# MoayedHajiAli/ElasticDiffusion-official

Hardware: AMD Instinct MI355X
Metric: images/sec at 50 steps (SDXL 2048x1024) (higher is better)
Workload: dtype fp16

## Files before the change

elasticdiffusion_official_amd/_hip.py:

```python
import ctypes
import os
import subprocess

import torch

PKG_DIR = os.path.dirname(os.path.abspath(__file__))
ROOT_DIR = os.path.dirname(PKG_DIR)
SOURCES = [os.path.join(PKG_DIR, "csrc", n) for n in ("elastic_kernels.hip", "unet_kernels.hip", "attention_kernels.hip", "gemm_kernels.hip", "vae_kernels.hip",
                                                       "canny_kernels.hip", "resize_kernels.hip", "mask_kernels.hip", "lora_kernels.hip")]
SRC = SOURCES[0]
INCLUDE = os.path.join(ROOT_DIR, "include")
SO_PATH = os.path.join(PKG_DIR, "libelastic_hip.so")
ABI_VERSION = 13

HIPCC_FLAGS = ["--offload-arch=gfx950", "-O3", "-std=c++17", "-ffp-contract=off", "-fPIC", "-shared"]

_i32p = ctypes.POINTER(ctypes.c_int32)
_vp, _i, _f, _i64 = ctypes.c_void_p, ctypes.c_int, ctypes.c_float, ctypes.c_int64

SIGNATURES = {
    "ed_version": [],
    "ed_error_string": [_i],
    "ed_gather_views": [_vp, _vp, _i, _i, _i, _i, _i, _vp, _vp, _i, _i, _i, _i, _i, _i, _i, _vp, _f, _vp],
    "ed_scatter_centres": [_vp, _i, _vp, _i, _i, _i, _i, _i, _i, _i, _vp, _vp, _vp, _vp, _vp],
# ... 21 lines not shown
    "ed_groupnorm_nhwc_cat": [_vp, _vp, _vp, _vp, _vp, _vp, _i, _i, _i, _i, _i, _i, _f, _i, _vp],
    "ed_assemble_rows": [_vp, _i, _i, _i, _i, _vp, _vp, _vp, _vp, _vp, _vp, _i, _i, _i, _i, _i, _i, _i, _vp, _vp, _vp, _vp,
                         _i, _i, _i, _i, _i, _i, _i, _i, _vp],
    "ed_assemble_rows_x": [_vp, _i, _i, _i, _i, _vp, _vp, _vp, _vp, _vp, _vp, _i, _i, _i, _i, _i, _i, _i, _vp, _vp, _vp, _vp,
                           _i, _i, _i, _i, _i, _i, _i, _i, _vp, _i, _vp, _vp],
    "ed_phase_epilogue": [_vp, _vp, _i, _vp, _vp, _vp, _vp, _vp, _vp, _vp, _vp, _vp, _vp, _vp, _vp, _vp, _vp, _vp, _vp, _vp,
                          _vp, _vp, _vp, _i, _i, _i, _i, _i, _i, _i, _i, _i, _i, _i, _i, _i, _i, _f, _f, _f, _f, _f, _f, _f,
                          _vp],
    "ed_softmax_rows": [_vp, _i64, _i64, _f, _vp],
    "ed_groupnorm_f32": [_vp, _vp, _vp, _vp, _vp, _i, _i, _i, _i, _f, _i, _vp],
    "ed_groupnorm_f32_workspace": [_i, _i, _i, _i],
    "ed_flash_attention": [_vp, _vp, _vp, _vp, _i, _i, _i, _i, _i, _i, _i64, _i64, _i64, _i64, _i64, _i64, _i64, _i64, _f, _i, _vp],
    "ed_geglu_gemm": [_vp, _vp, _vp, _vp, _i, _i64, _i, _i, _vp],
    "ed_linear": [_vp, _vp, _vp, _vp, _vp, _i, _i64, _i, _i, _vp],
    "ed_conv3x3_nhwc": [_vp, _vp, _vp, _vp, _vp, _vp, _i, _i, _i, _i, _i, _i, _vp],
    "ed_conv3x3_nhwc_up2x": [_vp, _vp, _vp, _vp, _i, _i, _i, _i, _i, _i, _vp],
    "ed_conv3x3_nhwc_s2": [_vp, _vp, _vp, _vp, _i, _i, _i, _i, _i, _i, _vp],
    "ed_absmax_f32": [_vp, _i64, _vp, _vp],
    "ed_split_f32_nhwc": [_vp, _vp, _i, _i, _i, _i, _i, _vp, _vp],
    "ed_groupnorm_nhwc_f32_workspace": [_i, _i, _i, _i],
    "ed_groupnorm_nhwc_f32": [_vp, _vp, _vp, _vp, _vp, _i, _i, _i, _i, _f, _i, _i, _vp],
    "ed_conv3x3_nhwc_f32out": [_vp, _vp, _vp, _vp, _vp, _i, _i, _i, _i, _i, _i, _f, _vp, _vp],
    "ed_conv3x3_nhwc_f32out_s2": [_vp, _vp, _vp, _vp, _i, _i, _i, _i, _i, _i, _f, _vp, _vp],
    "ed_canny_workspace": [_i, _i, _i],
    "ed_canny_map": [_vp, _i, _i, _i, _i, _i, _vp, _vp],
    "ed_canny_hysteresis": [_vp, _i, _i, _vp, _vp, _vp],
    "ed_canny_edges": [_vp, _i, _i, _vp, _vp, _vp],
    "ed_cfg_ddim_step_pt": [_vp, _vp, _vp, _vp, _vp, _f, _f, _f, _f, _f, _i64, _i, _vp],
    "ed_rrg_update_pt": [_vp, _vp, _vp, _vp, _vp, _vp, _vp, _vp, _f, _f, _f, _f, _f, _i, _i, _i, _i, _i, _i, _i, _vp],
    "ed_phase_epilogue_pt": [_vp, _vp, _i, _vp, _vp, _vp, _vp, _vp, _vp, _vp, _vp, _vp, _vp, _vp, _vp, _vp, _vp, _vp, _vp,
# ... 81 lines not shown
```

elasticdiffusion_official_amd/csrc/gemm_kernels.hip:

```cpp
#include <hip/hip_runtime.h>
#include <stdint.h>
#include <stdlib.h>

#include "elastic_hip.h"

namespace {

typedef float f32x4 __attribute__((ext_vector_type(4)));
typedef __bf16 bf16x8 __attribute__((ext_vector_type(8)));
typedef _Float16 f16x8 __attribute__((ext_vector_type(8)));
typedef uint32_t u32x4 __attribute__((ext_vector_type(4)));
typedef __attribute__((address_space(3))) void* lds_ptr_t;

struct BF {
  typedef bf16x8 v8;
  static __device__ __forceinline__ f32x4 mfma(v8 a, v8 b, f32x4 c) {
    return __builtin_amdgcn_mfma_f32_16x16x32_bf16(a, b, c, 0, 0, 0);
  }
  static __device__ __forceinline__ float to_f32(uint16_t h) { return __builtin_bit_cast(float, (uint32_t)h << 16); }
  static __device__ __forceinline__ uint16_t from_f32(float f) { return __builtin_bit_cast(uint16_t, (__bf16)f); }
  static __device__ __forceinline__ uint32_t pack2(float lo, float hi) {
    typedef float f2 __attribute__((ext_vector_type(2)));
    typedef __bf16 b2 __attribute__((ext_vector_type(2)));
    return __builtin_bit_cast(uint32_t, __builtin_convertvector(f2{lo, hi}, b2));
// ... 85 lines not shown
  ++p.tile;
  if (CONV) {
    ++p.tap;
    p.w += cpt;
    if (p.tap == 9) {
      p.tap = 0;
      ++p.ct;
      p.w = p.ct;
    }
  } else {
    p.w = p.tile;
  }
  return p;
}

template <int BUFI, int CONV>
__device__ __forceinline__ void stage_x(uint8_t* lds, const Ctx& c, KPos p, int h) {
  const int rg = (c.wave & 3) + 8 * (c.wave >> 2) + 4 * h;
  uint8_t* dst = lds + BUFI * BUF + x_sub(0, 0) + rg * (2 * SUB);
  if (CONV) {
    const int dy = p.tap / 3 - 1, dx = p.tap - 3 * (p.tap / 3) - 1;
    int delta;
    if (CONV == CONV_UP2X) {
      const int yp = (c.px_mask[h] >> 16) & 1, xp = (c.px_mask[h] >> 17) & 1;
      delta = (((yp + dy) >> 1) * c.img_w + ((xp + dx) >> 1)) * c.cin2 + p.ct * (BK * 2);
    } else {
      delta = (dy * c.img_w + dx) * c.cin2 + p.ct * (BK * 2);
    }
    const int vo = ((c.px_mask[h] >> p.tap) & 1) ? c.x_voff[h] + delta : (int)0x80000000;
    __builtin_amdgcn_raw_ptr_buffer_load_lds(c.xr, (lds_ptr_t)dst, 16, vo, 0, 0, 0);
// ... 159 lines not shown
  ED_BARRIER();
  read_w<T, BUFI, 1>(lds, c, f);
  if (s2) {
    stage_w<BUFI>(lds, c, p2.w, 0);
    stage_x<BUFI, CONV>(lds, c, p2, 0);
    ED_WAIT_VM(4);
  } else {
    ED_WAIT_VM(0);
  }
  ED_WAIT_LGKM(0);
  ED_BARRIER();
  mma16<T, 0, 1>(acc, f);
  ED_BARRIER();
}

template <class T, int EPI, int CONV, bool ADD = true, bool OUT32 = false, bool TWO = false, bool ROWS = false>
__global__ void __launch_bounds__(512, 2)
k_gemm_8phase(const uint16_t* __restrict__ x, const uint16_t* __restrict__ w, const uint16_t* __restrict__ bias,
              const uint16_t* __restrict__ row_bias, const uint16_t* __restrict__ residual, uint16_t* __restrict__ out, int M,
              int K, int I, int n_blocks_n, int n_blocks, int img_h, int img_w, int rows_per_sample, float out_scale,
              const float* __restrict__ act_absmax) {
  __shared__ __attribute__((aligned(1024))) uint8_t lds[2 * BUF];

  const int bid = blockIdx.x;
  const int q = n_blocks >> 3, r = n_blocks & 7, xcd = bid & 7;
  const int tid = (xcd < r ? xcd * (q + 1) : r * (q + 1) + (xcd - r) * q) + (bid >> 3);
  const int n_blocks_m = n_blocks / n_blocks_n;
  const int per_group = 8 * n_blocks_n, grp = tid / per_group, first = grp * 8;
  const int rows_here = n_blocks_m - first < 8 ? n_blocks_m - first : 8;
  constexpr int TBM = ROWS ? BM / 2 : BM;
  constexpr int WROWS = TBM / 2;
  constexpr int NMB = WROWS / 16;
  const int m0 = (first + (tid % per_group) % rows_here) * TBM;
  const int n0 = ((tid % per_group) / rows_here) * (EPI == 0 ? BN : 2 * BN);
  const int gap = EPI == 0 ? I : BN;

  const int lane = threadIdx.x & 63;
  Ctx c;
  c.wave = __builtin_amdgcn_readfirstlane(threadIdx.x >> 6);
// ... 51 lines not shown

  const int ncol = n0 + 32 * wcol + 8 * (lane >> 4);
  u32x4 bias_v = {0, 0, 0, 0}, bias_g = {0, 0, 0, 0};
  if (bias && !OUT32) {
    if (EPI == 0 || ncol < I) bias_v = *reinterpret_cast<const u32x4*>(bias + ncol);
    if (EPI == 0 || ncol + gap < I) bias_g = *reinterpret_cast<const u32x4*>(bias + gap + ncol);
  }

  f32x4 acc[8][4];
#pragma unroll
  for (int a = 0; a < 8; ++a)
#pragma unroll
    for (int b = 0; b < 4; ++b) acc[a][b] = f32x4{0.f, 0.f, 0.f, 0.f};
  Frags<T> f;

  const int nt = K / BK;
  const KPos p0 = {0, 0, 0, 0};
  KPos pa = k_next<CONV>(p0, c.cpt);
  KPos pb = k_next<CONV>(pa, c.cpt);
  const bool half = !ROWS && EPI == 1 && n0 + BN >= I;
  if (ROWS) {
    stage_w<0>(lds, c, 0, 0);
    stage_x<0, CONV>(lds, c, p0, 0);
    stage_w<0>(lds, c, 0, 1);
    if (nt > 1) {
      stage_w<1>(lds, c, pa.w, 0);
      stage_x<1, CONV>(lds, c, pa, 0);
      ED_WAIT_VM(4);
    } else {
      ED_WAIT_VM(0);
    }
    ED_BARRIER();
    if (wrow == 1) ED_BARRIER();
    int tr = 0;
    for (; tr + 1 < nt; tr += 2) {
      tile_phases_rows<T, 0, CONV>(lds, c, f, acc, true, tr + 2 < nt, pa, pb);
      pa = pb;
      pb = k_next<CONV>(pb, c.cpt);
      tile_phases_rows<T, 1, CONV>(lds, c, f, acc, tr + 2 < nt, tr + 3 < nt, pa, pb);
      pa = pb;
      pb = k_next<CONV>(pb, c.cpt);
    }
    if (tr < nt) tile_phases_rows<T, 0, CONV>(lds, c, f, acc, false, false, pa, pb);
    if (wrow == 0) ED_BARRIER();
  } else if (half) {
    stage_w<0>(lds, c, 0, 0);
    stage_x<0, CONV>(lds, c, p0, 0);
    stage_x<0, CONV>(lds, c, p0, 1);
    if (nt > 1) {
      stage_w<1>(lds, c, pa.w, 0);
      stage_x<1, CONV>(lds, c, pa, 0);
      ED_WAIT_VM(4);
    } else {
      ED_WAIT_VM(0);
    }
    ED_BARRIER();
    if (wrow == 1) ED_BARRIER();
    int th = 0;
    for (; th + 1 < nt; th += 2) {
      tile_phases_half<T, 0, CONV>(lds, c, f, acc, th, true, th + 2 < nt, pa, pb);
      pa = pb;
      pb = k_next<CONV>(pb, c.cpt);
      tile_phases_half<T, 1, CONV>(lds, c, f, acc, th + 1, th + 2 < nt, th + 3 < nt, pa, pb);
      pa = pb;
      pb = k_next<CONV>(pb, c.cpt);
    }
    if (th < nt) tile_phases_half<T, 0, CONV>(lds, c, f, acc, th, false, false, pa, pb);
    if (wrow == 0) ED_BARRIER();
  } else {
  stage_w<0>(lds, c, 0, 0);
  stage_x<0, CONV>(lds, c, p0, 0);
  stage_w<0>(lds, c, 0, 1);
  stage_x<0, CONV>(lds, c, p0, 1);
  constexpr bool two = TWO;
  const bool early = nt >= 3 && !two;
  if (nt > 1) {
    stage_w<1>(lds, c, pa.w, 0);
    stage_x<1, CONV>(lds, c, pa, 0);
    stage_w<1>(lds, c, pa.w, 1);
    if (early) ED_WAIT_VM(10);
    else ED_WAIT_VM(6);
  } else {
    ED_WAIT_VM(0);
  }
  ED_BARRIER();
  if (wrow == 1) ED_BARRIER();

// ... 19 lines not shown
    pb = k_next<CONV>(pb, c.cpt);
    t = 2;
  }
  for (; t + 1 < nt; t += 2) {
    tile_phases<T, 0, CONV>(lds, c, f, acc, t, true, t + 2 < nt, pa, pb);
    pa = pb;
    pb = k_next<CONV>(pb, c.cpt);
    tile_phases<T, 1, CONV>(lds, c, f, acc, t + 1, t + 2 < nt, t + 3 < nt, pa, pb);
    pa = pb;
    pb = k_next<CONV>(pb, c.cpt);
  }
  if (t < nt) tile_phases<T, 0, CONV>(lds, c, f, acc, t, false, false, pa, pb);
  if (wrow == 0) ED_BARRIER();
  }

  if (OUT32) {
    const float* biasf = reinterpret_cast<const float*>(bias);
    const float* resf = reinterpret_cast<const float*>(residual);
    float* outf = reinterpret_cast<float*>(out);
    if (act_absmax) {
      const int E = (int)((__builtin_bit_cast(uint32_t, *act_absmax) >> 23) & 0xffu) - 127;
      const int e = E > 14 ? E - 14 : 0;
      out_scale *= __builtin_bit_cast(float, (uint32_t)(127 + e) << 23);
    }
    const bool col_v = ncol < I, col_g = ncol + gap < I;
    f32x4 b32[2][2] = {{f32x4{0.f, 0.f, 0.f, 0.f}, f32x4{0.f, 0.f, 0.f, 0.f}}, {f32x4{0.f, 0.f, 0.f, 0.f}, f32x4{0.f, 0.f, 0.f, 0.f}}};
    if (biasf) {
#pragma unroll
      for (int fr = 0; fr < 2; ++fr) {
        if (col_v) b32[0][fr] = *reinterpret_cast<const f32x4*>(biasf + ncol + 4 * fr);
// ... 204 lines not shown
#pragma unroll
        for (int jj = 0; jj < 2; ++jj) {
          const float o0 = geglu_one(acc[mb][nf][2 * jj] + bv[nf][2 * jj], acc[mb][2 + nf][2 * jj] + bg[nf][2 * jj]);
          const float o1 = geglu_one(acc[mb][nf][2 * jj + 1] + bv[nf][2 * jj + 1], acc[mb][2 + nf][2 * jj + 1] + bg[nf][2 * jj + 1]);
          pk[nf * 2 + jj] = T::pack2(o0, o1);
        }
      if (m < M) *reinterpret_cast<u32x4*>(out + (int64_t)m * I + ncol) = u32x4{pk[0], pk[1], pk[2], pk[3]};
    }
    if (!has_next) break;
    bid = next, tp = tp2, c = c2;
  }
}

}

static int gemm_cus() {
  static int cus[16] = {0};
  int dev = 0;
  if (hipGetDevice(&dev) != hipSuccess || dev < 0 || dev >= 16) return 0;
  if (cus[dev] == 0) {
    int n = 0;
    if (hipDeviceGetAttribute(&n, hipDeviceAttributeMultiprocessorCount, dev) != hipSuccess || n < 8) return 0;
    cus[dev] = n / 8 * 8;
  }
  return cus[dev];
}
constexpr double ROWS_TILE_COST = 0.72;

template <int EPI, int CONV, bool OUT32 = false>
static int launch(const void* x, const void* w, const void* bias, const void* row_bias, const void* residual, void* out, int dtype,
                  int64_t M, int K, int I, int img_h, int img_w, int rows_per_sample, void* stream, float out_scale = 1.0f,
                  const float* act_absmax = nullptr) {
  if (M == 0) return 0;
  const int bad = (int)hipErrorInvalidValue;
  if (M < 0 || K % BK != 0 || K < BK || I <= 0 || (EPI == 0 ? I % BN != 0 : I % 8 != 0)) return bad;
  if (CONV && (K % (9 * BK) != 0 || img_h <= 0 || img_w <= 0 || M % ((int64_t)img_h * img_w) != 0)) return bad;
  if (CONV == CONV_UP2X && (img_h % 2 != 0 || img_w % 2 != 0 || row_bias || residual)) return bad;
  if (CONV >= CONV_S2 && (row_bias || residual || 4 * M * (int64_t)(K / 9) * 2 >= 0x7ffffff0ll)) return bad;
  if (row_bias && (rows_per_sample <= 0 || M % rows_per_sample != 0)) return bad;
  if (M * (int64_t)(CONV ? K / 9 : K) * 2 >= 0x7ffffff0ll || (int64_t)(EPI == 0 ? 2 : 1) * I * K * 2 >= 0x7ffffff0ll) return bad;
  if ((((uintptr_t)x | (uintptr_t)w | (uintptr_t)out | (uintptr_t)bias | (uintptr_t)row_bias | (uintptr_t)residual) & 15u)) return bad;
  const int nbn = EPI == 0 ? I / BN : (I + 2 * BN - 1) / (2 * BN);
  const int64_t nb256 = ((M + BM - 1) / BM) * nbn, nb128 = ((M + BM / 2 - 1) / (BM / 2)) * nbn;
  if (nb128 >= (1ll << 31) || M >= (1ll << 31)) return bad;
  hipStream_t s = (hipStream_t)stream;
  const bool add = EPI == 1 && (row_bias || residual);
  const bool two = CONV && K / BK >= TWO_MIN_TILES;
  bool rows = false;
  if (!OUT32 && EPI == 1 && CONV < CONV_UP2X) {
    const int cus = gemm_cus();
    const double r256 = (double)((nb256 + cus - 1) / cus), r128 = (double)((nb128 + cus - 1) / cus) * ROWS_TILE_COST;
    rows = cus > 0 && r128 < r256 - 1e-9;
    if (const char* e = getenv("ED_GEMM_ROWS")) rows = e[0] == '1' ? true : (e[0] == '0' ? false : rows);
  }
  const int64_t nb = rows ? nb128 : nb256;
#define ED_LAUNCH1(TT, ADD_, TWO_, ROWS_)                                                                                            \
  k_gemm_8phase<TT, EPI, CONV, ADD_, OUT32, TWO_, ROWS_><<<(int)nb, 512, 0, s>>>((const uint16_t*)x, (const uint16_t*)w, (const uint16_t*)bias, \
                                                             (const uint16_t*)row_bias, (const uint16_t*)residual, (uint16_t*)out,  \
                                                             (int)M, K, I, nbn, (int)nb, img_h, img_w, rows_per_sample > 0 ? rows_per_sample : 1, out_scale, \
                                                             act_absmax)
#define ED_LAUNCH(TT, ADD_)                                   \
  do {                                                        \
    if constexpr (OUT32 || EPI == 0) {                        \
      if constexpr (CONV) {                                   \
        if (two) ED_LAUNCH1(TT, ADD_, true, false);           \
        else ED_LAUNCH1(TT, ADD_, false, false);              \
      } else {                                                \
        ED_LAUNCH1(TT, ADD_, false, false);                   \
      }                                                       \
    } else if (CONV < CONV_UP2X && rows) {                    \
      if constexpr (CONV < CONV_UP2X) ED_LAUNCH1(TT, ADD_, false, true);   \
    } else if constexpr (CONV) {                              \
      if (two) ED_LAUNCH1(TT, ADD_, true, false);             \
      else ED_LAUNCH1(TT, ADD_, false, false);                \
    } else {                                                  \
// ... 79 lines not shown
int ed_conv3x3_nhwc_f32out(const void* x, const void* w, const float* bias, const float* residual, float* out, int dtype, int B, int H, int W,
                           int Cin, int N, float out_scale, const float* act_absmax, void* stream) {
  if (B < 0 || H <= 0 || W <= 0 || Cin <= 0 || ((uintptr_t)act_absmax & 3u)) return (int)hipErrorInvalidValue;
  return launch<1, 1, true>(x, w, bias, nullptr, residual, out, dtype, (int64_t)B * H * W, 9 * Cin, N, H, W, H * W, stream, out_scale,
                               act_absmax);
}

int ed_conv3x3_nhwc_f32out_s2(const void* x, const void* w, const float* bias, float* out, int dtype, int B, int H, int W, int Cin, int N,
                              float out_scale, const float* act_absmax, void* stream) {
  if (B < 0 || H <= 0 || W <= 0 || Cin <= 0 || ((uintptr_t)act_absmax & 3u)) return (int)hipErrorInvalidValue;
  return launch<1, CONV_S2P0, true>(x, w, bias, nullptr, nullptr, out, dtype, (int64_t)B * H * W, 9 * Cin, N, H, W, H * W, stream, out_scale,
                                    act_absmax);
}

}
```

elasticdiffusion_official_amd/models.py:

```python
import math
import os
from types import SimpleNamespace

import torch
import torch.nn as nn
import torch.nn.functional as F

from . import ops


FUSED_KERNELS = True


CHANNELS_LAST = os.environ.get("ED_CHANNELS_LAST", "1") == "1"


_HALF = (torch.bfloat16, torch.float16)


def _fusable(x):
    return FUSED_KERNELS and x.is_cuda and x.dtype in _HALF and x.is_contiguous()


def _fusable_nhwc(x):
# ... 68 lines not shown


FUSED_LAYERNORM = True
FUSED_TEMB_ADD = True
FUSED_CONV_BIAS = True
FUSED_ADD_LAYERNORM = True
FUSED_TOKENS_ADD = True
FLASH_ATTENTION = True
FUSED_QKV = True
HIP_GEGLU_GEMM = True
HIP_LINEAR = True
FUSED_SKIP_CAT = True
FUSED_PROJ_OUT_ADD = True
HIP_DOWNSAMPLE_CONV = False
FUSED_RESIDUAL_LINEAR = False
FUSED_UPSAMPLE_CONV = True
HIP_CONV3X3 = True
VAE_HIP_GROUPNORM = True
VAE_HIP_ATTENTION = True
VAE_NCHW_RESIDUAL = True
VAE_SPLIT_CONV = True
VAE_SPLIT_DOWNSAMPLE = True
for _name in filter(None, os.environ.get("ED_DISABLE", "").split(",")):
    if _name not in globals() or not isinstance(globals()[_name], bool):
        raise RuntimeError(f"ED_DISABLE: unknown switch {_name!r}")
    globals()[_name] = False


def fused_unet_entry_points():
    hip_conv = FUSED_KERNELS and HIP_CONV3X3 and CHANNELS_LAST
    on = [("ed_groupnorm_nhwc" if CHANNELS_LAST else "ed_groupnorm", FUSED_KERNELS),
          ("ed_geglu_gemm" if HIP_GEGLU_GEMM else "ed_geglu", FUSED_KERNELS),
          ("ed_layernorm", FUSED_KERNELS and FUSED_LAYERNORM),
          ("ed_flash_attention", FUSED_KERNELS and FLASH_ATTENTION),
          ("ed_add_layernorm", FUSED_KERNELS and FUSED_ADD_LAYERNORM),
          ("ed_tokens_add_nchw", FUSED_KERNELS and FUSED_TOKENS_ADD and not CHANNELS_LAST),
          ("ed_bias_residual_add", FUSED_KERNELS and FUSED_CONV_BIAS and FUSED_TEMB_ADD and not hip_conv)]
    return {n for n, flag in on if flag}


def linear_(x, weight, bias=None):
    if (HIP_LINEAR and FUSED_KERNELS and _fusable(x) and weight.dtype == x.dtype and weight.is_contiguous()
            and ops.linear_wins(x.numel() // x.shape[-1], x.shape[-1], weight.shape[0])):
        return ops.linear(x, weight, bias)
    return F.linear(x, weight, bias)


def linear_res_(x, weight, bias, residual):
    if (FUSED_RESIDUAL_LINEAR and residual is not None and HIP_LINEAR and FUSED_KERNELS and _fusable(x) and _fusable(residual)
            and weight.dtype == x.dtype == residual.dtype and weight.is_contiguous()
            and residual.shape == x.shape[:-1] + (weight.shape[0],)
            and ops.linear_wins(x.numel() // x.shape[-1], x.shape[-1], weight.shape[0])):
        return ops.linear(x, weight, bias, residual=residual), True
    return linear_(x, weight, bias), False


# ... 131 lines not shown
        sc, c1, c2 = self.conv_shortcut, self.conv1, self.conv2
        cout = c1.out_channels
        if _stream32(x, c1.weight.dtype):
            def add_to_stream(h):
                if sc is None:
                    return x + h
                xs = x.to(h.dtype)
                return (_shortcut_nhwc(sc, xs) if ops.is_nhwc(xs) else sc(xs)).float() + h

            def close(a2):
                B, _, H, W = a2.shape
                if a2.dtype == torch.float16 and ops.conv3x3_f32out_ok(B, H, W, cout, cout):
                    res = x if sc is None else _shortcut_nhwc(sc, x.to(a2.dtype)).float()
                    res = res.contiguous(memory_format=torch.channels_last)
                    return ops.conv3x3_f32out(a2, c2.weight, _f32_bias(c2), res, 1.0)
                return add_to_stream(ops.conv3x3_nhwc(a2, c2.weight, c2.bias))

            a = group_norm_act(self.norm1, x, silu=True)
            if _hip_conv_pair(self, a, a.shape[1]):
                return self._hip_convs(a, tb, close)
            return add_to_stream(c2(group_norm_act(self.norm2, c1(a), silu=True, chan_bias=tb)))
        cl = _fusable_nhwc(x) and cout % 8 == 0 and cout // self.norm2.num_groups >= 8
        if x.shape[1] // self.norm1.num_groups >= 8 and _hip_conv_pair(self, x, x.shape[1]):
            return self._hip_convs(group_norm_act(self.norm1, x, silu=True), tb, lambda a2: ops.conv3x3_nhwc(
                a2, c2.weight, c2.bias, residual=x if sc is None else _shortcut_nhwc(sc, x)))
        if FUSED_CONV_BIAS and FUSED_TEMB_ADD and (cl or (_fusable(x) and (x.shape[2] * x.shape[3]) % 8 == 0)):
            h = F.conv2d(group_norm_act(self.norm1, x, silu=True), c1.weight, None, padding=1)
            a = group_norm_act(self.norm2, h, silu=True, chan_bias=tb, conv_bias=c1.bias)
            h = F.conv2d(a, c2.weight, None, padding=1)
            if sc is None:
                return ops.bias_residual_add(h, c2.bias, x)
            if cl:
                res = F.linear(x.permute(0, 2, 3, 1), sc.weight.reshape(cout, -1)).permute(0, 3, 1, 2)
            else:
                res = F.conv2d(x, sc.weight, None)
            return ops.bias_residual_add(h, c2.bias, res, sc.bias)
        h = c1(group_norm_act(self.norm1, x, silu=True))
        a = group_norm_act(self.norm2, h, silu=True, chan_bias=tb)
        if sc is not None and SHORTCUT_AS_GEMM and _fusable(x):
            N, C, H, W = x.shape
            h = F.conv2d(a, c2.weight, c2.bias + sc.bias, padding=1)
            w = sc.weight.view(1, cout, C).expand(N, -1, -1)
            return torch.baddbmm(h.view(N, cout, H * W), w, x.view(N, C, H * W)).view(N, cout, H, W)
        return (x if sc is None else sc(x)) + c2(a)

    def _hip_convs(self, a, tb, close):
        h = ops.conv3x3_nhwc(a, self.conv1.weight, self.conv1.bias, sample_bias=None if tb is None else tb.contiguous())
        return close(group_norm_act(self.norm2, h, silu=True))

    def forward_cat(self, x, skip, temb=None):
        sc, c2 = self.conv_shortcut, self.conv2
        C1, C = x.shape[1], x.shape[1] + skip.shape[1]
        if (FUSED_SKIP_CAT and FUSED_KERNELS and sc is not None and _fusable_nhwc(skip) and x.dtype == skip.dtype
                and _hip_conv_pair(self, x, C) and ops.groupnorm_nhwc_cat_ok(x, skip, self.norm1.num_groups)
                and self.conv1.weight.shape[1] == C and sc.weight.dtype == x.dtype):
            def close(a2):
                w1, w2 = _split_shortcut(sc, C1)
                xt, st = x.permute(0, 2, 3, 1), skip.permute(0, 2, 3, 1)
                y = linear_(xt, w1, sc.bias)
                M, cout = st.numel() // st.shape[-1], w2.shape[0]
                if HIP_LINEAR and ops.linear_wins(M, st.shape[-1], cout):
                    y = ops.linear(st, w2, None, residual=y)
                else:
                    y = torch.addmm(y.reshape(M, cout), st.reshape(M, -1), w2.t()).view(y.shape)
                return ops.conv3x3_nhwc(a2, c2.weight, c2.bias, residual=y.permute(0, 3, 1, 2))

            tb = self.time_emb_proj(F.silu(temb)) if self.time_emb_proj is not None else None
            n1 = self.norm1
            return self._hip_convs(ops.groupnorm_nhwc_cat(x, skip, n1.weight, n1.bias, n1.num_groups, n1.eps, silu=True), tb, close)
        return self(torch.cat([x, skip], dim=1), temb)

    def _forward_split(self, x):
        n1, n2, sc = self.norm1, self.norm2, self.conv_shortcut
        _, cin, H, W = x.shape

        def block(xs):
            w1, s1 = _split_weight(self.conv1)
            w2, s2 = _split_weight(self.conv2)
            a = ops.groupnorm_nhwc_f32(xs, n1.weight, n1.bias, n1.num_groups, n1.eps, silu=True, split=True)
            h = ops.conv3x3_f32out(a, w1, self.conv1.bias, None, s1)
# ... 689 lines not shown
```

elasticdiffusion_official_amd/ops.py:

```python
import torch

from . import _hip

ED_F32, ED_F16, ED_BF16 = 0, 1, 2
_DTYPE = {torch.float32: ED_F32, torch.float16: ED_F16, torch.bfloat16: ED_BF16}


_LAUNCH = {"device": None}


def _stream_of(t):
    if _LAUNCH["device"] is None:
        _LAUNCH["device"] = t.device
    return _stream()


def _stream():
    dev = _LAUNCH["device"]
    if dev is None:
        raise RuntimeError("internal: _stream() before any device tensor argument")
    return torch.cuda.current_stream(dev).cuda_stream


class KernelTimer:
# ... 574 lines not shown
        return None
    ncb = -(-N // (2 * GEMM_BN))
    tps = HW // GEMM_BM * ncb
    total = B * tps

    def rounds(tiles):
        return min(-(-tiles // GEMM_CUS), -(-2 * tiles // GEMM_CUS) * GEMM_ROWS_TILE_COST)

    full = total // GEMM_CUS
    if full < 3 or total % GEMM_CUS == 0:
        return None
    BA = full * GEMM_CUS // tps
    if BA <= 0 or BA >= B:
        return None
    return BA if -(-BA * tps // GEMM_CUS) + rounds((B - BA) * tps) < rounds(total) - 0.1 else None


def conv3x3_up2x_wins(B, H, W, Cin, N):
    ncb = -(-N // (2 * GEMM_BN))
    return (H % 2 == 0 and W % 2 == 0 and conv3x3_wins(B, H, W, Cin, N) and not gemm_rows_mode(B * H * W, ncb)
            and B * (H // 2) * (W // 2) * Cin * 2 < 2 ** 31 - 16)


def conv3x3_nhwc_up2x(x, w, bias=None):
    if not (isinstance(x, torch.Tensor) and x.is_cuda and x.dim() == 4 and x.dtype in (torch.float16, torch.bfloat16)):
        _reject("conv3x3_nhwc_up2x: x must be a 16-bit [B,C,H,W] tensor on the MI355X; no CPU fallback")
    B, Cin, Hs, Ws = x.shape
    H, W = 2 * Hs, 2 * Ws
    N = w.shape[0]
    cl = torch.channels_last
# ... 830 lines not shown
```

include/elastic_hip.h:

```cpp
#ifndef ELASTIC_HIP_H
#define ELASTIC_HIP_H

#include <stdint.h>

#ifdef __cplusplus
extern "C" {
#endif

enum { ED_F32 = 0, ED_F16 = 1, ED_BF16 = 2 };

enum { ED_PRED_EPSILON = 0, ED_PRED_V = 1 };

int ed_version(void);

const char* ed_error_string(int err);

int ed_gather_views(const float* latent, void* out, int dtype, int B, int C, int H, int W,
                    const int32_t* win_y0, const int32_t* win_x0, int V, int Sh, int Sw,
                    int PH, int PW, int off_y, int off_x, const float* frame, float divisor, void* stream);

int ed_scatter_centres(const void* pred, int dtype, float* local, int B, int C, int H, int W,
                       int PH, int PW, int n_col_blocks,
                       const int32_t* row_blk, const int32_t* row_src,
                       const int32_t* col_blk, const int32_t* col_src, void* stream);
// ... 149 lines not shown

int64_t ed_groupnorm_f32_workspace(int N, int C, int HW, int G);
int ed_groupnorm_f32(const void* x, const void* gamma, const void* beta, void* out, float* workspace, int N, int C, int HW,
                     int G, float eps, int act_silu, void* stream);

int ed_softmax_rows(void* x, int64_t rows, int64_t cols, float scale, void* stream);

int ed_geglu_gemm(const void* x, const void* w, const void* bias, void* out, int dtype, int64_t M, int K, int I, void* stream);

int ed_linear(const void* x, const void* w, const void* bias, const void* residual, void* out, int dtype, int64_t M, int K, int N,
              void* stream);

int ed_conv3x3_nhwc(const void* x, const void* w, const void* bias, const void* sample_bias, const void* residual, void* out,
                    int dtype, int B, int H, int W, int Cin, int N, void* stream);

int ed_conv3x3_nhwc_up2x(const void* x, const void* w, const void* bias, void* out, int dtype, int B, int H, int W, int Cin, int N,
                         void* stream);

int ed_conv3x3_nhwc_s2(const void* x, const void* w, const void* bias, void* out, int dtype, int B, int H, int W, int Cin, int N,
                       void* stream);

int ed_absmax_f32(const void* x, int64_t n, float* out, void* stream);
int ed_split_f32_nhwc(const void* x, void* out, int N, int C, int H, int W, int upsample2x, const float* absmax, void* stream);
int64_t ed_groupnorm_nhwc_f32_workspace(int N, int C, int HW, int G);
int ed_groupnorm_nhwc_f32(const void* x, const void* gamma, const void* beta, void* out, float* workspace, int N, int C, int HW, int G,
                          float eps, int act_silu, int split16, void* stream);
int ed_conv3x3_nhwc_f32out(const void* x, const void* w, const float* bias, const float* residual, float* out, int dtype, int B, int H, int W,
                           int Cin, int N, float out_scale, const float* act_absmax, void* stream);

int ed_conv3x3_nhwc_f32out_s2(const void* x, const void* w, const float* bias, float* out, int dtype, int B, int H, int W, int Cin, int N,
// ... 41 lines not shown
```

Before: 0.1023.

## Split-K the partial last wave of GEMM and conv3x3 tiles

Adds a split-K path for linear and 3x3 conv GEMMs. Full waves of output tiles run as before, and the leftover partial wave is split across K slices that write fp32 partial sums to a workspace. A finish kernel then reduces the slices and applies bias, per-sample bias and residual. A cost model decides when to split, aiming to fill idle CUs in the tail wave, at the cost of extra launches, workspace traffic and a per-call allocation.

```diff
diff --git a/elasticdiffusion_official_amd/_hip.py b/elasticdiffusion_official_amd/_hip.py
--- a/elasticdiffusion_official_amd/_hip.py
+++ b/elasticdiffusion_official_amd/_hip.py
@@ -7,7 +7,7 @@
 PKG_DIR = os.path.dirname(os.path.abspath(__file__))
 ROOT_DIR = os.path.dirname(PKG_DIR)
 SOURCES = [os.path.join(PKG_DIR, "csrc", n) for n in ("elastic_kernels.hip", "unet_kernels.hip", "attention_kernels.hip", "gemm_kernels.hip", "vae_kernels.hip",
-                                                       "canny_kernels.hip", "resize_kernels.hip", "mask_kernels.hip", "lora_kernels.hip")]
+                                                       "canny_kernels.hip", "resize_kernels.hip", "mask_kernels.hip", "lora_kernels.hip", "gemm_ksplit_kernels.hip")]
 SRC = SOURCES[0]
 INCLUDE = os.path.join(ROOT_DIR, "include")
 SO_PATH = os.path.join(PKG_DIR, "libelastic_hip.so")
@@ -59,6 +59,8 @@
     "ed_geglu_gemm": [_vp, _vp, _vp, _vp, _i, _i64, _i, _i, _vp],
     "ed_linear": [_vp, _vp, _vp, _vp, _vp, _i, _i64, _i, _i, _vp],
     "ed_conv3x3_nhwc": [_vp, _vp, _vp, _vp, _vp, _vp, _i, _i, _i, _i, _i, _i, _vp],
+    "ed_linear_ksplit": [_vp, _vp, _vp, _vp, _vp, _i, _i64, _i, _i, _i64, _i, _vp, _i64, _vp],
+    "ed_conv3x3_nhwc_ksplit": [_vp, _vp, _vp, _vp, _vp, _vp, _i, _i, _i, _i, _i, _i, _i64, _i, _vp, _i64, _vp],
     "ed_conv3x3_nhwc_up2x": [_vp, _vp, _vp, _vp, _i, _i, _i, _i, _i, _i, _vp],
     "ed_conv3x3_nhwc_s2": [_vp, _vp, _vp, _vp, _i, _i, _i, _i, _i, _i, _vp],
     "ed_absmax_f32": [_vp, _i64, _vp, _vp],
diff --git a/elasticdiffusion_official_amd/csrc/gemm_kernels.hip b/elasticdiffusion_official_amd/csrc/gemm_kernels.hip
--- a/elasticdiffusion_official_amd/csrc/gemm_kernels.hip
+++ b/elasticdiffusion_official_amd/csrc/gemm_kernels.hip
@@ -123,6 +123,15 @@
   return p;
 }
 
+template <int CONV>
+__device__ __forceinline__ KPos kpos_at(int tile, int cpt) {
+  if (CONV) {
+    const int ct = tile / 9, tap = tile - 9 * ct;
+    return KPos{tile, tap, ct, tap * cpt + ct};
+  }
+  return KPos{tile, 0, 0, tile};
+}
+
 template <int BUFI, int CONV>
 __device__ __forceinline__ void stage_x(uint8_t* lds, const Ctx& c, KPos p, int h) {
   const int rg = (c.wave & 3) + 8 * (c.wave >> 2) + 4 * h;
@@ -312,15 +321,22 @@
   ED_BARRIER();
 }
 
-template <class T, int EPI, int CONV, bool ADD = true, bool OUT32 = false, bool TWO = false, bool ROWS = false>
+template <class T, int EPI, int CONV, bool ADD = true, bool OUT32 = false, bool TWO = false, bool ROWS = false, bool KS = false>
 __global__ void __launch_bounds__(512, 2)
 k_gemm_8phase(const uint16_t* __restrict__ x, const uint16_t* __restrict__ w, const uint16_t* __restrict__ bias,
               const uint16_t* __restrict__ row_bias, const uint16_t* __restrict__ residual, uint16_t* __restrict__ out, int M,
               int K, int I, int n_blocks_n, int n_blocks, int img_h, int img_w, int rows_per_sample, float out_scale,
-              const float* __restrict__ act_absmax) {
+              const float* __restrict__ act_absmax, int ks_from, int ks_tail, int ks_slices) {
   __shared__ __attribute__((aligned(1024))) uint8_t lds[2 * BUF];
 
-  const int bid = blockIdx.x;
+  int bid = blockIdx.x;
+  int kt0 = 0, nt = K / BK;
+  if (KS) {
+    const int slice = bid / ks_tail, base = nt / ks_slices, rem = nt - base * ks_slices;
+    bid = ks_from + (bid - slice * ks_tail);
+    kt0 = slice * base + (slice < rem ? slice : rem);
+    nt = base + (slice < rem ? 1 : 0);
+  }
   const int q = n_blocks >> 3, r = n_blocks & 7, xcd = bid & 7;
   const int tid = (xcd < r ? xcd * (q + 1) : r * (q + 1) + (xcd - r) * q) + (bid >> 3);
   const int n_blocks_m = n_blocks / n_blocks_n;
@@ -402,15 +418,14 @@
     for (int b = 0; b < 4; ++b) acc[a][b] = f32x4{0.f, 0.f, 0.f, 0.f};
   Frags<T> f;
 
-  const int nt = K / BK;
-  const KPos p0 = {0, 0, 0, 0};
+  const KPos p0 = kpos_at<CONV>(kt0, c.cpt);
   KPos pa = k_next<CONV>(p0, c.cpt);
   KPos pb = k_next<CONV>(pa, c.cpt);
   const bool half = !ROWS && EPI == 1 && n0 + BN >= I;
   if (ROWS) {
-    stage_w<0>(lds, c, 0, 0);
+    stage_w<0>(lds, c, p0.w, 0);
     stage_x<0, CONV>(lds, c, p0, 0);
-    stage_w<0>(lds, c, 0, 1);
+    stage_w<0>(lds, c, p0.w, 1);
     if (nt > 1) {
       stage_w<1>(lds, c, pa.w, 0);
       stage_x<1, CONV>(lds, c, pa, 0);
@@ -432,7 +447,7 @@
     if (tr < nt) tile_phases_rows<T, 0, CONV>(lds, c, f, acc, false, false, pa, pb);
     if (wrow == 0) ED_BARRIER();
   } else if (half) {
-    stage_w<0>(lds, c, 0, 0);
+    stage_w<0>(lds, c, p0.w, 0);
     stage_x<0, CONV>(lds, c, p0, 0);
     stage_x<0, CONV>(lds, c, p0, 1);
     if (nt > 1) {
@@ -456,9 +471,9 @@
     if (th < nt) tile_phases_half<T, 0, CONV>(lds, c, f, acc, th, false, false, pa, pb);
     if (wrow == 0) ED_BARRIER();
   } else {
-  stage_w<0>(lds, c, 0, 0);
+  stage_w<0>(lds, c, p0.w, 0);
   stage_x<0, CONV>(lds, c, p0, 0);
-  stage_w<0>(lds, c, 0, 1);
+  stage_w<0>(lds, c, p0.w, 1);
   stage_x<0, CONV>(lds, c, p0, 1);
   constexpr bool two = TWO;
   const bool early = nt >= 3 && !two;
@@ -508,6 +523,20 @@
   if (wrow == 0) ED_BARRIER();
   }
 
+  if (KS) {
+    float* ws = reinterpret_cast<float*>(out) + (int64_t)blockIdx.x * (BM * 2 * BN);
+#pragma unroll
+    for (int mb = 0; mb < NMB; ++mb) {
+      float* row = ws + (WROWS * wrow + 16 * mb + (lane & 15)) * (2 * BN) + 32 * wcol + 8 * (lane >> 4);
+#pragma unroll
+      for (int hf = 0; hf < 2; ++hf) {
+        if (hf == 1 && half) continue;
+#pragma unroll
+        for (int fr = 0; fr < 2; ++fr) *reinterpret_cast<f32x4*>(row + hf * BN + 4 * fr) = acc[mb][2 * hf + fr];
+      }
+    }
+    return;
+  }
   if (OUT32) {
     const float* biasf = reinterpret_cast<const float*>(bias);
     const float* resf = reinterpret_cast<const float*>(residual);
@@ -742,6 +771,7 @@
 
 }
 
+#ifndef ED_GEMM_DEVICE_CODE_ONLY
 static int gemm_cus() {
   static int cus[16] = {0};
   int dev = 0;
@@ -758,7 +788,7 @@
 template <int EPI, int CONV, bool OUT32 = false>
 static int launch(const void* x, const void* w, const void* bias, const void* row_bias, const void* residual, void* out, int dtype,
                   int64_t M, int K, int I, int img_h, int img_w, int rows_per_sample, void* stream, float out_scale = 1.0f,
-                  const float* act_absmax = nullptr) {
+                  const float* act_absmax = nullptr, int64_t first_tiles = -1) {
   if (M == 0) return 0;
   const int bad = (int)hipErrorInvalidValue;
   if (M < 0 || K % BK != 0 || K < BK || I <= 0 || (EPI == 0 ? I % BN != 0 : I % 8 != 0)) return bad;
@@ -781,12 +811,16 @@
     rows = cus > 0 && r128 < r256 - 1e-9;
     if (const char* e = getenv("ED_GEMM_ROWS")) rows = e[0] == '1' ? true : (e[0] == '0' ? false : rows);
   }
+  if (first_tiles >= 0) rows = false;
   const int64_t nb = rows ? nb128 : nb256;
+  if (first_tiles > nb) return bad;
+  const int64_t grid = first_tiles >= 0 ? first_tiles : nb;
+  if (grid == 0) return 0;
 #define ED_LAUNCH1(TT, ADD_, TWO_, ROWS_)                                                                                            \
-  k_gemm_8phase<TT, EPI, CONV, ADD_, OUT32, TWO_, ROWS_><<<(int)nb, 512, 0, s>>>((const uint16_t*)x, (const uint16_t*)w, (const uint16_t*)bias, \
+  k_gemm_8phase<TT, EPI, CONV, ADD_, OUT32, TWO_, ROWS_><<<(int)grid, 512, 0, s>>>((const uint16_t*)x, (const uint16_t*)w, (const uint16_t*)bias, \
                                                              (const uint16_t*)row_bias, (const uint16_t*)residual, (uint16_t*)out,  \
                                                              (int)M, K, I, nbn, (int)nb, img_h, img_w, rows_per_sample > 0 ? rows_per_sample : 1, out_scale, \
-                                                             act_absmax)
+                                                             act_absmax, 0, 1, 1)
 #define ED_LAUNCH(TT, ADD_)                                   \
   do {                                                        \
     if constexpr (OUT32 || EPI == 0) {                        \
@@ -896,3 +930,11 @@
 }
 
 }
+
+int ed_gemm_first_tiles(int conv, const void* x, const void* w, const void* bias, const void* row_bias, const void* residual, void* out,
+                        int dtype, int64_t M, int K, int I, int img_h, int img_w, int rows_per_sample, int64_t first_tiles, void* stream) {
+  if (first_tiles < 0) return (int)hipErrorInvalidValue;
+  return conv ? launch<1, 1>(x, w, bias, row_bias, residual, out, dtype, M, K, I, img_h, img_w, rows_per_sample, stream, 1.0f, nullptr, first_tiles)
+              : launch<1, 0>(x, w, bias, row_bias, residual, out, dtype, M, K, I, img_h, img_w, rows_per_sample, stream, 1.0f, nullptr, first_tiles);
+}
+#endif
diff --git a/elasticdiffusion_official_amd/csrc/gemm_ksplit_kernels.hip b/elasticdiffusion_official_amd/csrc/gemm_ksplit_kernels.hip
--- /dev/null
+++ b/elasticdiffusion_official_amd/csrc/gemm_ksplit_kernels.hip
@@ -0,0 +1,109 @@
+#define ED_GEMM_DEVICE_CODE_ONLY
+#include "gemm_kernels.hip"
+
+int ed_gemm_first_tiles(int conv, const void* x, const void* w, const void* bias, const void* row_bias, const void* residual, void* out,
+                        int dtype, int64_t M, int K, int I, int img_h, int img_w, int rows_per_sample, int64_t first_tiles, void* stream);
+
+namespace {
+
+template <class T>
+__global__ void __launch_bounds__(256)
+k_ksplit_finish(const float* __restrict__ ws, const uint16_t* __restrict__ bias, const uint16_t* __restrict__ row_bias,
+                const uint16_t* __restrict__ residual, uint16_t* __restrict__ out, int M, int I, int n_blocks_n, int n_blocks,
+                int rows_per_sample, int ks_from, int ks_tail, int ks_slices) {
+  const int j = blockIdx.x >> 5;
+  const int bid = ks_from + j;
+  const int q = n_blocks >> 3, r = n_blocks & 7, xcd = bid & 7;
+  const int tid = (xcd < r ? xcd * (q + 1) : r * (q + 1) + (xcd - r) * q) + (bid >> 3);
+  const int n_blocks_m = n_blocks / n_blocks_n;
+  const int per_group = 8 * n_blocks_n, grp = tid / per_group, first = grp * 8;
+  const int rows_here = n_blocks_m - first < 8 ? n_blocks_m - first : 8;
+  const int m0 = (first + (tid % per_group) % rows_here) * BM;
+  const int n0 = ((tid % per_group) / rows_here) * (2 * BN);
+  const int lr = (blockIdx.x & 31) * 8 + (threadIdx.x >> 5), lc = (threadIdx.x & 31) * 8;
+  const int m = m0 + lr, n = n0 + lc;
+  if (m >= M || n >= I) return;
+  const float* p = ws + ((int64_t)j * BM + lr) * (2 * BN) + lc;
+  const int64_t slice_stride = (int64_t)ks_tail * (BM * 2 * BN);
+  f32x4 a0 = *reinterpret_cast<const f32x4*>(p), a1 = *reinterpret_cast<const f32x4*>(p + 4);
+  for (int s = 1; s < ks_slices; ++s) {
+    a0 += *reinterpret_cast<const f32x4*>(p + s * slice_stride);
+    a1 += *reinterpret_cast<const f32x4*>(p + s * slice_stride + 4);
+  }
+  const int64_t o = (int64_t)m * I + n;
+  u32x4 bv = {0, 0, 0, 0}, rv = {0, 0, 0, 0}, sv = {0, 0, 0, 0};
+  if (bias) bv = *reinterpret_cast<const u32x4*>(bias + n);
+  if (row_bias) rv = *reinterpret_cast<const u32x4*>(row_bias + (int64_t)(m / rows_per_sample) * I + n);
+  if (residual) sv = *reinterpret_cast<const u32x4*>(residual + o);
+  uint32_t pk[4];
+#pragma unroll
+  for (int e = 0; e < 8; e += 2) {
+    float v0 = (e < 4 ? a0[e] : a1[e - 4]) + T::to_f32((uint16_t)bv[e >> 1]);
+    float v1 = (e < 4 ? a0[e + 1] : a1[e - 3]) + T::to_f32((uint16_t)(bv[e >> 1] >> 16));
+    v0 += T::to_f32((uint16_t)rv[e >> 1]), v1 += T::to_f32((uint16_t)(rv[e >> 1] >> 16));
+    v0 += T::to_f32((uint16_t)sv[e >> 1]), v1 += T::to_f32((uint16_t)(sv[e >> 1] >> 16));
+    pk[e >> 1] = (uint32_t)T::from_f32(v0) | ((uint32_t)T::from_f32(v1) << 16);
+  }
+  *reinterpret_cast<u32x4*>(out + o) = u32x4{pk[0], pk[1], pk[2], pk[3]};
+}
+
+}
+
+template <int CONV>
+static int launch_ksplit(const void* x, const void* w, const void* bias, const void* row_bias, const void* residual, void* out, int dtype,
+                         int64_t M, int K, int I, int img_h, int img_w, int rows_per_sample, int64_t split_from_tile, int slices,
+                         void* workspace, int64_t workspace_bytes, void* stream) {
+  const int bad = (int)hipErrorInvalidValue;
+  if (M <= 0 || K % BK != 0 || K < BK || I <= 0 || I % 8 != 0 || (dtype != ED_BF16 && dtype != ED_F16)) return bad;
+  const int nbn = (I + 2 * BN - 1) / (2 * BN);
+  const int64_t nb = ((M + BM - 1) / BM) * nbn;
+  if (nb >= (1ll << 31) || split_from_tile < 0 || split_from_tile >= nb || slices < 1) return bad;
+  const int64_t tail = nb - split_from_tile;
+  if (K / BK / slices < 2 || tail * slices >= (1ll << 26)) return bad;
+  if (!workspace || ((uintptr_t)workspace & 15u) || workspace_bytes < tail * slices * (int64_t)(BM * 2 * BN * 4)) return bad;
+  hipStream_t s = (hipStream_t)stream;
+  const int e = ed_gemm_first_tiles(CONV, x, w, bias, row_bias, residual, out, dtype, M, K, I, img_h, img_w, rows_per_sample, split_from_tile,
+                                    stream);
+  if (e != 0) return e;
+  const bool two = CONV && K / BK >= TWO_MIN_TILES;
+  const int rps = rows_per_sample > 0 ? rows_per_sample : 1;
+#define ED_KS(TT, TWO_)                                                                                                               \
+  k_gemm_8phase<TT, 1, CONV, false, false, TWO_, false, true><<<(int)(tail * slices), 512, 0, s>>>(                                   \
+      (const uint16_t*)x, (const uint16_t*)w, nullptr, nullptr, nullptr, (uint16_t*)workspace, (int)M, K, I, nbn, (int)nb, img_h, img_w, rps, \
+      1.0f, nullptr, (int)split_from_tile, (int)tail, slices)
+#define ED_KS_LAUNCH(TT)                    \
+  do {                                      \
+    if constexpr (CONV) {                   \
+      if (two) ED_KS(TT, true);             \
+      else ED_KS(TT, false);                \
+    } else {                                \
+      ED_KS(TT, false);                     \
+    }                                       \
+    k_ksplit_finish<TT><<<(int)(tail * 32), 256, 0, s>>>((const float*)workspace, (const uint16_t*)bias, (const uint16_t*)row_bias,   \
+                                                         (const uint16_t*)residual, (uint16_t*)out, (int)M, I, nbn, (int)nb, rps,       \
+                                                         (int)split_from_tile, (int)tail, slices);                                      \
+  } while (0)
+  if (dtype == ED_BF16) ED_KS_LAUNCH(BF);
+  else ED_KS_LAUNCH(HF);
+#undef ED_KS_LAUNCH
+#undef ED_KS
+  return (int)hipGetLastError();
+}
+
+extern "C" {
+
+int ed_linear_ksplit(const void* x, const void* w, const void* bias, const void* residual, void* out, int dtype, int64_t M, int K, int N,
+                     int64_t split_from_tile, int slices, void* workspace, int64_t workspace_bytes, void* stream) {
+  return launch_ksplit<0>(x, w, bias, nullptr, residual, out, dtype, M, K, N, 0, 0, 0, split_from_tile, slices, workspace, workspace_bytes,
+                          stream);
+}
+
+int ed_conv3x3_nhwc_ksplit(const void* x, const void* w, const void* bias, const void* sample_bias, const void* residual, void* out,
+                           int dtype, int B, int H, int W, int Cin, int N, int64_t split_from_tile, int slices, void* workspace,
+                           int64_t workspace_bytes, void* stream) {
+  if (B <= 0 || H <= 0 || W <= 0 || Cin <= 0) return (int)hipErrorInvalidValue;
+  return launch_ksplit<1>(x, w, bias, sample_bias, residual, out, dtype, (int64_t)B * H * W, 9 * Cin, N, H, W, H * W, split_from_tile,
+                          slices, workspace, workspace_bytes, stream);
+}
+
+}
diff --git a/elasticdiffusion_official_amd/models.py b/elasticdiffusion_official_amd/models.py
--- a/elasticdiffusion_official_amd/models.py
+++ b/elasticdiffusion_official_amd/models.py
@@ -106,6 +106,8 @@
 FUSED_PROJ_OUT_ADD = True
 HIP_DOWNSAMPLE_CONV = False
 FUSED_RESIDUAL_LINEAR = False
+KSPLIT_TAIL = True
+KSPLIT_TAIL_LINEAR = True
 FUSED_UPSAMPLE_CONV = True
 HIP_CONV3X3 = True
 VAE_HIP_GROUPNORM = True
@@ -131,7 +133,25 @@
     return {n for n, flag in on if flag}
 
 
+def _linear_ksplit_plan(x, weight):
+    M, K, N = x.numel() // x.shape[-1], x.shape[-1], weight.shape[0]
+    if not (KSPLIT_TAIL_LINEAR and K > 1280 and M > 0 and ops.linear_ok(M, K, N)) or ops.linear_wins(M, K, N):
+        return None
+    return ops.ksplit_plan(-(-M // ops.GEMM_BM) * -(-N // (2 * ops.GEMM_BN)), K // 64)
+
+
+def conv3x3_(x, weight, bias=None, sample_bias=None, residual=None):
+    plan = ops.conv3x3_ksplit_plan(x.shape[0], x.shape[2], x.shape[3], x.shape[1], weight.shape[0]) if KSPLIT_TAIL else None
+    if plan is not None:
+        return ops.conv3x3_nhwc_ksplit(x, weight, bias, sample_bias=sample_bias, residual=residual, split_from_tile=plan[0], slices=plan[1])
+    return ops.conv3x3_nhwc(x, weight, bias, sample_bias=sample_bias, residual=residual)
+
+
 def linear_(x, weight, bias=None):
+    if HIP_LINEAR and FUSED_KERNELS and KSPLIT_TAIL_LINEAR and _fusable(x) and weight.dtype == x.dtype and weight.is_contiguous():
+        plan = _linear_ksplit_plan(x, weight)
+        if plan is not None:
+            return ops.linear_ksplit(x, weight, bias, split_from_tile=plan[0], slices=plan[1])
     if (HIP_LINEAR and FUSED_KERNELS and _fusable(x) and weight.dtype == x.dtype and weight.is_contiguous()
             and ops.linear_wins(x.numel() // x.shape[-1], x.shape[-1], weight.shape[0])):
         return ops.linear(x, weight, bias)
@@ -293,7 +313,7 @@
                     res = x if sc is None else _shortcut_nhwc(sc, x.to(a2.dtype)).float()
                     res = res.contiguous(memory_format=torch.channels_last)
                     return ops.conv3x3_f32out(a2, c2.weight, _f32_bias(c2), res, 1.0)
-                return add_to_stream(ops.conv3x3_nhwc(a2, c2.weight, c2.bias))
+                return add_to_stream(conv3x3_(a2, c2.weight, c2.bias))
 
             a = group_norm_act(self.norm1, x, silu=True)
             if _hip_conv_pair(self, a, a.shape[1]):
@@ -301,7 +321,7 @@
             return add_to_stream(c2(group_norm_act(self.norm2, c1(a), silu=True, chan_bias=tb)))
         cl = _fusable_nhwc(x) and cout % 8 == 0 and cout // self.norm2.num_groups >= 8
         if x.shape[1] // self.norm1.num_groups >= 8 and _hip_conv_pair(self, x, x.shape[1]):
-            return self._hip_convs(group_norm_act(self.norm1, x, silu=True), tb, lambda a2: ops.conv3x3_nhwc(
+            return self._hip_convs(group_norm_act(self.norm1, x, silu=True), tb, lambda a2: conv3x3_(
                 a2, c2.weight, c2.bias, residual=x if sc is None else _shortcut_nhwc(sc, x)))
         if FUSED_CONV_BIAS and FUSED_TEMB_ADD and (cl or (_fusable(x) and (x.shape[2] * x.shape[3]) % 8 == 0)):
             h = F.conv2d(group_norm_act(self.norm1, x, silu=True), c1.weight, None, padding=1)
@@ -324,7 +344,7 @@
         return (x if sc is None else sc(x)) + c2(a)
 
     def _hip_convs(self, a, tb, close):
-        h = ops.conv3x3_nhwc(a, self.conv1.weight, self.conv1.bias, sample_bias=None if tb is None else tb.contiguous())
+        h = conv3x3_(a, self.conv1.weight, self.conv1.bias, sample_bias=None if tb is None else tb.contiguous())
         return close(group_norm_act(self.norm2, h, silu=True))
 
     def forward_cat(self, x, skip, temb=None):
@@ -342,7 +362,7 @@
                     y = ops.linear(st, w2, None, residual=y)
                 else:
                     y = torch.addmm(y.reshape(M, cout), st.reshape(M, -1), w2.t()).view(y.shape)
-                return ops.conv3x3_nhwc(a2, c2.weight, c2.bias, residual=y.permute(0, 3, 1, 2))
+                return conv3x3_(a2, c2.weight, c2.bias, residual=y.permute(0, 3, 1, 2))
 
             tb = self.time_emb_proj(F.silu(temb)) if self.time_emb_proj is not None else None
             n1 = self.norm1
diff --git a/elasticdiffusion_official_amd/ops.py b/elasticdiffusion_official_amd/ops.py
--- a/elasticdiffusion_official_amd/ops.py
+++ b/elasticdiffusion_official_amd/ops.py
@@ -612,6 +612,93 @@
     if BA <= 0 or BA >= B:
         return None
     return BA if -(-BA * tps // GEMM_CUS) + rounds((B - BA) * tps) < rounds(total) - 0.1 else None
+
+
+KSPLIT_TILE_FIXED = 4.7
+KSPLIT_SLICE_COST = 4.7
+KSPLIT_FINISH_COST = 12.0
+KSPLIT_SLICE_SLOWDOWN = 1.2
+KSPLIT_MAX_SLICES = 8
+KSPLIT_MIN_SLICE_TILES = 4
+KSPLIT_MARGIN = 0.1
+KSPLIT_CONV_MIN_FULL_ROUNDS = 3
+
+
+def ksplit_ranges(k_tiles, slices):
+    base, rem = divmod(k_tiles, slices)
+    return [(s * base + min(s, rem), (s + 1) * base + min(s + 1, rem)) for s in range(slices)]
+
+
+def ksplit_plan(tiles, k_tiles):
+    full, tail = divmod(tiles, GEMM_CUS)
+    if full < 2 or tail == 0:
+        return None
+    slices = min(KSPLIT_MAX_SLICES, GEMM_CUS // tail)
+    if slices < 2 or k_tiles // slices < KSPLIT_MIN_SLICE_TILES:
+        return None
+    today = 1.0 if full < 3 else min(1.0, -(-2 * tail // GEMM_CUS) * GEMM_ROWS_TILE_COST)
+    split = (KSPLIT_SLICE_SLOWDOWN * -(-k_tiles // slices) + KSPLIT_SLICE_COST
+             + KSPLIT_FINISH_COST * tail * slices / GEMM_CUS) / (k_tiles + KSPLIT_TILE_FIXED)
+    return (full * GEMM_CUS, slices) if split < today - KSPLIT_MARGIN else None
+
+
+def _ksplit_workspace(tiles, split_from_tile, slices, like, what):
+    if not (isinstance(split_from_tile, int) and isinstance(slices, int) and 0 <= split_from_tile < tiles and slices >= 1):
+        _reject(f"{what}: split_from_tile {split_from_tile!r} / slices {slices!r} outside a grid of {tiles} tiles")
+    n = (tiles - split_from_tile) * slices
+    if n > (1 << 16):
+        _reject(f"{what}: {n} slices of partial sums")
+    return torch.empty((n, GEMM_BM, 2 * GEMM_BN), dtype=torch.float32, device=like.device)
+
+
+def linear_ksplit(x, w, bias=None, residual=None, split_from_tile=0, slices=2):
+    M, K = _gemm_x(x, "x")
+    N = w.shape[0]
+    if tuple(w.shape) != (N, K) or not linear_ok(M, K, N) or M == 0:
+        _reject(f"linear_ksplit: unsupported shape x {tuple(x.shape)} w {tuple(w.shape)}")
+    if isinstance(slices, int) and slices >= 1 and K // 64 // slices < 2:
+        _reject(f"linear_ksplit: {slices} slices of K = {K} are shorter than 2 K tiles")
+    out = torch.empty(x.shape[:-1] + (N,), dtype=x.dtype, device=x.device)
+    if residual is not None and (residual.shape != out.shape or residual.dtype != x.dtype):
+        _reject("linear_ksplit: residual must match the output")
+    ws = _ksplit_workspace(-(-M // GEMM_BM) * -(-N // (2 * GEMM_BN)), split_from_tile, slices, x, "linear_ksplit")
+    TIMER.note_work("ed_linear_ksplit", flops=2.0 * M * K * N, nbytes=2.0 * (M * K + N * K + M * N * (2 if residual is not None else 1)))
+    _call("ed_linear_ksplit", _dev(x, None, "x"), _dev(w, x.dtype, "w"), _opt(bias, x.dtype, "bias"), _opt(residual, x.dtype, "residual"),
+          _dev(out, None, "out"), _code(x, "x"), M, K, N, split_from_tile, slices, ws.data_ptr(), ws.numel() * 4, _stream())
+    return out
+
+
+def conv3x3_nhwc_ksplit(x, w, bias=None, sample_bias=None, residual=None, split_from_tile=0, slices=2):
+    if not (isinstance(x, torch.Tensor) and x.is_cuda and x.dim() == 4 and x.dtype in (torch.float16, torch.bfloat16)):
+        _reject("conv3x3_nhwc_ksplit: x must be a 16-bit [B,C,H,W] tensor on the MI355X; no CPU fallback")
+    B, Cin, H, W = x.shape
+    N = w.shape[0]
+    cl = torch.channels_last
+    if tuple(w.shape) != (N, Cin, 3, 3) or w.dtype != x.dtype or not conv3x3_ok(B, H, W, Cin, N) or B == 0:
+        _reject(f"conv3x3_nhwc_ksplit: unsupported shape x {tuple(x.shape)} w {tuple(w.shape)}")
+    if not x.is_contiguous(memory_format=cl) or not w.is_contiguous(memory_format=cl):
+        _reject("conv3x3_nhwc_ksplit: x and w must be channels_last")
+    if isinstance(slices, int) and slices >= 1 and 9 * Cin // 64 // slices < 2:
+        _reject(f"conv3x3_nhwc_ksplit: {slices} slices of K = {9 * Cin} are shorter than 2 K tiles")
+    out = torch.empty((B, N, H, W), dtype=x.dtype, device=x.device, memory_format=cl)
+    if residual is not None and (residual.shape != out.shape or residual.dtype != x.dtype or not residual.is_contiguous(memory_format=cl)):
+        _reject("conv3x3_nhwc_ksplit: residual must be a channels_last tensor of the output's shape")
+    if sample_bias is not None and tuple(sample_bias.shape) != (B, N):
+        _reject("conv3x3_nhwc_ksplit: sample_bias must be [B, N]")
+    ws = _ksplit_workspace(-(-(B * H * W) // GEMM_BM) * -(-N // (2 * GEMM_BN)), split_from_tile, slices, x, "conv3x3_nhwc_ksplit")
+    TIMER.note_work("ed_conv3x3_nhwc_ksplit", flops=2.0 * B * H * W * 9 * Cin * N,
+                    nbytes=2.0 * (B * H * W * (Cin + N * (2 if residual is not None else 1)) + 9 * Cin * N))
+    _call("ed_conv3x3_nhwc_ksplit", x.data_ptr(), w.data_ptr(), _opt(bias, x.dtype, "bias"), _opt(sample_bias, x.dtype, "sample_bias"),
+          None if residual is None else residual.data_ptr(), out.data_ptr(), _code(x, "x"), B, H, W, Cin, N, split_from_tile, slices,
+          ws.data_ptr(), ws.numel() * 4, _stream_of(x))
+    return out
+
+
+def conv3x3_ksplit_plan(B, H, W, Cin, N):
+    tiles = -(-(B * H * W) // GEMM_BM) * -(-N // (2 * GEMM_BN))
+    if Cin % 64 or not conv3x3_ok(B, H, W, Cin, N) or tiles // GEMM_CUS < KSPLIT_CONV_MIN_FULL_ROUNDS:
+        return None
+    return ksplit_plan(tiles, 9 * Cin // 64)
 
 
 def conv3x3_up2x_wins(B, H, W, Cin, N):
diff --git a/include/elastic_hip.h b/include/elastic_hip.h
--- a/include/elastic_hip.h
+++ b/include/elastic_hip.h
@@ -187,6 +187,12 @@
 int ed_conv3x3_nhwc(const void* x, const void* w, const void* bias, const void* sample_bias, const void* residual, void* out,
                     int dtype, int B, int H, int W, int Cin, int N, void* stream);
 
+int ed_linear_ksplit(const void* x, const void* w, const void* bias, const void* residual, void* out, int dtype, int64_t M, int K, int N,
+                     int64_t split_from_tile, int slices, void* workspace, int64_t workspace_bytes, void* stream);
+int ed_conv3x3_nhwc_ksplit(const void* x, const void* w, const void* bias, const void* sample_bias, const void* residual, void* out,
+                           int dtype, int B, int H, int W, int Cin, int N, int64_t split_from_tile, int slices, void* workspace,
+                           int64_t workspace_bytes, void* stream);
+
 int ed_conv3x3_nhwc_up2x(const void* x, const void* w, const void* bias, void* out, int dtype, int B, int H, int W, int Cin, int N,
                          void* stream);
 
```

After: 0.1029, median of 6. About the same (+0.6%).
